# SunYangtian/UniGeo

Measured on AMD Instinct MI355X. Metric: frames/sec (384x512, 25-frame clip, 25 denoise steps), higher is better.
Workload: dtype fp16; 1 GPU; DepthCrafter SVD-UNet fp16, 25-step Euler, 25-frame 384x512 clips (BASELINE configs[1]); CLIP + VAE enc/dec + depth post-proc inside the timed region; one clip per ug_dc_run call, one call at a time (SURVEY 8d; reference eval.py:33-39); frames=25, height=384, width=512, denoise_steps=25, parallelism=clip-sharded x1, RCCL all_gather of depth, clips_in_flight_per_gpu=1, lanes=1

## Files before the change

### unigeo_amd/_lib.py

```python
import ctypes as C
import dataclasses
import json
import os

import numpy as np

_HERE = os.path.dirname(os.path.abspath(__file__))
LIB_PATH = os.environ.get("UG_LIB_PATH") or os.path.join(_HERE, "csrc", "libunigeo_hip.so")

EXPORTS = [
    "ug_unet_config_default", "ug_vae_config_default", "ug_clip_config_default",
    "ug_create", "ug_destroy", "ug_last_error", "ug_workspace_peak",
    "ug_load_tensor", "ug_bind_unet", "ug_bind_vae", "ug_bind_clip",
    "ug_dc_set_inputs", "ug_dc_run", "ug_dc_run_windows", "ug_dc_get_outputs", "ug_dc_device_ptrs", "ug_dc_set_trace", "ug_dc_set_guidance", "ug_unet_forward_pair", "ug_dc_set_inputs_ex", "ug_dc_get_noise", "ug_op_philox_u32", "ug_op_randn", "ug_op_u8_to_frames", "ug_set_vae_encode_fp32", "ug_set_concurrency", "ug_set_coscheduled", "ug_set_fp8_linears", "ug_op_linear_mx8", "ug_set_ff_fused", "ug_op_ff", "ug_op_ln_ff", "ug_bench_ff", "ug_bench_flash", "ug_tune_flash", "ug_tune_ff",
    "ug_eval_depth", "ug_eval_normal", "ug_depth_eval_opts_default", "ug_eval_depth_ex", "ug_eval_depth_global", "ug_op_masked_median", "ug_clip_embed", "ug_vae_encode", "ug_vae_decode", "ug_unet_forward", "ug_normals_from_depth",
    "ug_op_linear", "ug_op_conv", "ug_op_conv_gn", "ug_op_groupnorm", "ug_op_layernorm", "ug_op_flash_attn",
    "ug_op_temporal_attn", "ug_op_attention_generic", "ug_op_flash_attn_dh", "ug_op_euler_step", "ug_op_flash_cross_attn", "ug_op_temporal_attn_nv",
    "ug_op_split_pair", "ug_op_gn32_pair", "ug_op_conv_wide", "ug_op_attn_wide",
    "ug_bind_stablenormal", "ug_sn_run", "ug_sn_unet_forward", "ug_sn_dino", "ug_sn_vae_decode", "ug_sn_vae_encode", "ug_resize_bilinear",
    "ug_vis_depth_range", "ug_vis_panels", "ug_prep_resize_frames", "ug_prep_gt", "ug_prep_gt_ex",
    "ug_profile_begin", "ug_profile_begin_shapes", "ug_profile_end", "ug_bench_gemm", "ug_bench_groupnorm", "ug_bench_mfma_peak", "ug_tune_force",
]


class UNetConfigC(C.Structure):
    _fields_ = [("in_channels", C.c_int), ("out_channels", C.c_int), ("num_levels", C.c_int),
                ("block_out_channels", C.c_int * 8), ("num_attention_heads", C.c_int * 8),
                ("down_has_attn", C.c_int * 8),
                ("layers_per_block", C.c_int), ("cross_attention_dim", C.c_int),
                ("addition_time_embed_dim", C.c_int), ("projection_class_embeddings_input_dim", C.c_int),
                ("norm_groups", C.c_int),
# ... 89 lines not shown
    lib.ug_vae_decode.argtypes = [vp, vp, ip, ip, ip, vp]
    lib.ug_unet_forward.argtypes = [vp, vp, ip, ip, ip, C.c_float, vp, vp]
    lib.ug_normals_from_depth.argtypes = [vp, vp, vp, ip, ip, ip, vp]
    lib.ug_op_linear.argtypes = [vp, vp, ip, ip, vp, ip, vp, vp, C.c_float, C.c_float, ip, ip, vp]
    lib.ug_op_conv.argtypes = [vp, vp, ip, vp, ip, ip, ip, ip, vp, vp, ip, ip, ip, ip, ip, ip, ip, vp]
    lib.ug_op_groupnorm.argtypes = [vp, vp, ip, vp, ip, ip, ip, ip, C.c_float, ip, ip, vp, vp, vp]
    lib.ug_op_conv_gn.argtypes = [vp, vp, ip, ip, ip, ip, vp, vp, vp, ip, ip, ip, ip, C.c_float, ip, vp, vp, vp, vp, vp, vp]
    lib.ug_op_layernorm.argtypes = [vp, vp, ip, ip, C.c_float, vp, vp, vp, ip, vp, vp]
    lib.ug_op_flash_attn.argtypes = [vp, vp, ip, ip, ip, vp]
    lib.ug_op_temporal_attn.argtypes = [vp, vp, ip, ip, ip, vp]
    lib.ug_op_attention_generic.argtypes = [vp, vp, ip, ip, ip, ip, vp]
    lib.ug_op_flash_attn_dh.argtypes = [vp, vp, ip, ip, ip, ip, vp]
    lib.ug_op_euler_step.argtypes = [vp, vp, vp, C.c_long, C.c_float, C.c_float]
    _set_argtypes(lib, {"ug_op_flash_cross_attn": [vp, vp, vp, ip, ip, ip, ip, ip, C.c_long, C.c_long, C.c_long, C.c_long, vp],
                        "ug_op_temporal_attn_nv": [vp, vp, ip, ip, ip, ip, vp]})
    _set_argtypes(lib, {
        "ug_op_split_pair": [vp, vp, C.c_long, ip, vp, vp], "ug_op_gn32_pair": [vp, vp, ip, ip, ip, ip, C.c_float, ip, vp, vp, vp, vp],
        "ug_op_conv_wide": [vp, vp, ip, ip, ip, ip, vp, vp, ip, vp, ip, ip, ip, ip, ip, vp], "ug_op_attn_wide": [vp, vp, ip, ip, ip, vp]})
    lib.ug_bind_stablenormal.argtypes = [vp, C.POINTER(UNetConfigC), C.POINTER(VAEConfigC), C.POINTER(CLIPConfigC)]
    lib.ug_sn_run.argtypes = [vp, vp, ip, ip, ip, vp, C.c_float, ip, vp, vp, vp, vp]
    lib.ug_sn_unet_forward.argtypes = [vp, ip, vp, vp, ip, ip, ip, C.c_float, C.c_float, vp, vp, ip, vp]
    lib.ug_sn_dino.argtypes = [vp, vp, ip, ip, ip, vp]
    lib.ug_sn_vae_decode.argtypes = [vp, vp, ip, ip, ip, vp]
    lib.ug_sn_vae_encode.argtypes = [vp, vp, ip, ip, ip, vp]
    lib.ug_resize_bilinear.argtypes = [vp, vp, ip, ip, ip, ip, ip, ip, ip, vp]
    lib.ug_profile_begin.argtypes = [vp]
    lib.ug_bench_gemm.argtypes = [vp] + [ip] * 16 + [vp]
    lib.ug_bench_groupnorm.argtypes = [vp, ip, ip, ip, ip, ip, ip, ip, vp]
    lib.ug_bench_mfma_peak.argtypes = [vp, ip, vp]
    lib.ug_tune_force.argtypes = [vp, ip, ip]
# ... 496 lines not shown
        out = np.empty((M, N // 2 if geglu else N), np.float32)
        self._ck(self.lib.ug_op_linear(self.ctx, _ptr(A), M, K, _ptr(W), N, _ptr(b), _ptr(r), c0, c1, act, int(geglu), _ptr(out)))
        return out

    def op_conv(self, x0, weight, bias=None, x1=None, kt=1, k=3, stride=1, pad_t=1, pad_l=1, ups=1):
        x0 = _f32(x0); T, H, W, C0 = x0.shape
        x1a = None if x1 is None else _f32(x1); C1 = 0 if x1 is None else x1a.shape[-1]
        w = _f32(weight); O = w.shape[0]
        b = None if bias is None else _f32(bias)
        Ho, Wo = H * ups // stride, W * ups // stride
        out = np.empty((T, Ho, Wo, O), np.float32)
        self._ck(self.lib.ug_op_conv(self.ctx, _ptr(x0), C0, _ptr(x1a), C1, T, H, W, _ptr(w), _ptr(b), O, kt, k,
                                     stride, pad_t, pad_l, ups, _ptr(out)))
        return out

    def op_groupnorm(self, x0, G, eps, gamma, beta, x1=None, temporal=False, silu=False):
        x0 = _f32(x0); T, HW, C0 = x0.shape
        x1a = None if x1 is None else _f32(x1); C1 = 0 if x1 is None else x1a.shape[-1]
        out = np.empty((T, HW, C0 + C1), np.float32)
        self._ck(self.lib.ug_op_groupnorm(self.ctx, _ptr(x0), C0, _ptr(x1a), C1, T, HW, G, eps, int(temporal), int(silu),
                                          _ptr(_f32(gamma)), _ptr(_f32(beta)), _ptr(out)))
        return out

    def op_conv_gn(self, x, w, b, G, eps, gamma, beta, res=None, kt=1, k=3, temporal=False):
        x = _f32(x); T, H, W, C0 = x.shape; w = _f32(w); O = w.shape[0]
        r = None if res is None else _f32(res)
        co = np.empty((T, H, W, O), np.float32); y1 = np.empty_like(co); y2 = np.empty_like(co)
        rb = C.c_int(0)
        self._ck(self.lib.ug_op_conv_gn(self.ctx, _ptr(x), C0, T, H, W, _ptr(w), _ptr(None if b is None else _f32(b)), _ptr(r), O, kt, k, G, eps, int(temporal),
                                        _ptr(_f32(gamma)), _ptr(_f32(beta)), _ptr(co), _ptr(y1), _ptr(y2), C.byref(rb)))
# ... 109 lines not shown
```

### unigeo_amd/csrc/common.h

```cpp
#pragma once
#include <hip/hip_runtime.h>
#include <hip/hip_fp16.h>
#include <stdint.h>
#include <stdio.h>
#include <stdexcept>
#include <string>

typedef _Float16 f16;
typedef _Float16 f16x2 __attribute__((ext_vector_type(2)));
typedef _Float16 f16x4 __attribute__((ext_vector_type(4)));
typedef _Float16 f16x8 __attribute__((ext_vector_type(8)));
typedef float f32x4 __attribute__((ext_vector_type(4)));
typedef float f32x16 __attribute__((ext_vector_type(16)));

#define UG_CHECK(expr)                                                                        \
  do {                                                                                        \
    hipError_t _e = (expr);                                                                   \
    if (_e != hipSuccess)                                                                     \
      throw std::runtime_error(std::string(#expr) + " failed: " + hipGetErrorString(_e) +    \
                               " at " + __FILE__ + ":" + std::to_string(__LINE__));           \
  } while (0)

#define UG_REQUIRE(cond, msg)                                                                 \
  do {                                                                                        \
// ... 39 lines not shown
  int m_off;
  int group_m;
  int halo_tw, halo_lg;
  int tune_cfg_p1, tune_split_p1, tune_knobs;
  float2* stat_part; int stat_hw;
};
struct GemmTune { int cfg = -1, split = -1, knobs = 0; };
static inline void gemm_apply_tune(GemmP& p, const GemmTune& t) { p.tune_cfg_p1 = t.cfg + 1; p.tune_split_p1 = t.split + 1; p.tune_knobs = t.knobs; }
void launch_gemm_mx8(const GemmP& p, hipStream_t s);
void launch_quant_mx8(const f16* x, long ldx, long M, int K, unsigned char* q, unsigned* scales, long ld_s, hipStream_t s);
void launch_gemm(const GemmP& p, int batch, hipStream_t s, int* stat_rb = nullptr);
bool gemm_stream_supported(const GemmP& p, int batch);
void launch_gemm_stream(const GemmP& p, hipStream_t s);
bool conv_halo_supported(const GemmP& p, int batch, int bm, int bn);
void launch_conv_halo(const GemmP& p, int bm, int bn, hipStream_t s);
void gemm_plan(const GemmP& p, int batch, int* cfg_out, int* split_out);

struct FFusedP {
  const f16* X; const f16* W1; const f16* b1; const f16* W2; const f16* b2;
  const f16* R1; const f16* R2; float c0, c1, c2;
  f16* Out; int M, C; const f16* zero;
  const f16* ln_g; const f16* ln_b; float ln_eps; const f16* addvec; int rows_per_vec;
  int variant;
};
bool ff_fused_supported(int C);
void launch_ff_fused(const FFusedP& p, hipStream_t s);

struct GroupNormP {
  const f16* X0; const f16* X1; int C0, C1;
  int T, HW, G; float eps; int temporal; int silu;
// ... 131 lines not shown
```

### unigeo_amd/csrc/kernels/conv_halo.hip

```cpp
#include "gemm_common.h"
#include <algorithm>
#include <cstdlib>
#include <type_traits>

template <int BM, int BN, int LG, bool ST = false>
__global__ __launch_bounds__(12 * 64, 3) void conv_halo_kernel(const GemmP p) {
  constexpr int BK = 64, NCW = 8, WMW = 4, WNW = 2;
  constexpr unsigned SENT = 0x80000000u;
  constexpr int WTM = BM / WMW, WTN = BN / WNW;
  constexpr int MT = WTM / 16, NT = WTN / 16;
  constexpr int WID = 4 * NT;
  constexpr int LB = BN / 32;
  constexpr int WSLOT = BN * BK;
  constexpr int TW = 1 << LG, TH = BM >> LG;
  constexpr int PITCH = (TW + 2 + 7) & ~7;
  constexpr int GPR = PITCH / 8;
  constexpr int NG = (TH + 2) * GPR;
  constexpr int HALO = NG * 8 * BK;
  constexpr int HL = 2;
  constexpr int HSLOTS = 7 * HL;
  static_assert(TH * TW == BM && TW >= 16 && (NG + 3) / 4 <= HSLOTS, "tile geometry");
  static_assert((2 * HALO + 3 * WSLOT) * 2 <= 160 * 1024, "LDS");
  extern __shared__ __attribute__((aligned(16))) f16 smem[];
  f16* halo = smem;
  f16* ring = smem + 2 * HALO;

  const int tid = threadIdx.x, lane = tid & 63;
  const int wave = __builtin_amdgcn_readfirstlane(tid >> 6);
  const bool producer = wave >= NCW;
  const int ntn = (p.N + BN - 1) / BN, ntm = p.M / BM;
  const int ntiles = ntm * ntn;
  const int Cin = p.C0 + p.C1, nchunks = Cin / BK, nk = nchunks * 9;
  const int txn = p.Wo >> LG, tpf = (p.Ho / TH) * txn;

  const int nwg = gridDim.x, w = blockIdx.x;
  const TileWalk tw = tile_walk(p.flags, ntiles, nwg, w);
  const int my_tiles = tw.count;
  const int total_it = my_tiles * nk;

  auto tile_origin = [&](int tile, int& t, int& y0, int& x0, int& n0) {
    int tm, tn; tile_coord_p(p, tile, ntm, ntn, tm, tn);
    const int tmg = tm + p.m_off / BM;
    t = tmg / tpf;
    const int rem = tmg - t * tpf;
    const int tyi = rem / txn, txi = rem - tyi * txn;
    y0 = tyi * TH; x0 = txi * TW; n0 = tn * BN;
  };

  if (producer) {
    const int pw = wave - NCW;
    const int pc = lane & 7, lrow = lane >> 3;
    const int lc16_0 = (pc ^ ((0 + (lrow >> 1)) & 7)) * 16, lc16_1 = (pc ^ ((4 + (lrow >> 1)) & 7)) * 16;
    const int lc16_h = (pc ^ (((lrow >> 1) & 3) * 2)) * 16;
    const __amdgpu_buffer_rsrc_t rA0 = __builtin_amdgcn_make_buffer_rsrc((void*)p.A0, 0, (int)SENT, 0x00020000);
    const __amdgpu_buffer_rsrc_t rA1 = __builtin_amdgcn_make_buffer_rsrc((void*)(p.A1 ? p.A1 : p.A0), 0, (int)SENT, 0x00020000);
    const __amdgpu_buffer_rsrc_t rW = __builtin_amdgcn_make_buffer_rsrc((void*)p.W, 0, (int)SENT, 0x00020000);
    constexpr int ngw_max = (NG + 3) / 4;
    const int ngw = (NG - pw + 3) >> 2;
    int h_pix[HSLOTS];
    auto halo_setup = [&](int tile) {
      int t, y0, x0, n0; tile_origin(tile, t, y0, x0, n0);
#pragma unroll
      for (int k = 0; k < ngw_max; ++k) {
        const int grp = pw + 4 * k;
        const int hy = grp / GPR, hx = (grp - hy * GPR) * 8 + lrow;
        const int y = y0 - 1 + hy, x = x0 - 1 + hx;
        const bool ok = grp < NG && hx < TW + 2 && y >= 0 && y < p.Hi && x >= 0 && x < p.Wi;
        h_pix[k] = ok ? (t * p.Hi + y) * p.Wi + x : -1;
      }
    };
    auto halo_issue = [&](int k, int chunk, int hb) {
      const int cb = chunk * BK;
      const bool src0 = cb < p.C0;
      const int Cs2 = (src0 ? p.C0 : p.C1) * 2;
      const int soff = (src0 ? cb : cb - p.C0) * 2;
      const unsigned voff = h_pix[k] >= 0 ? (unsigned)h_pix[k] * (unsigned)Cs2 + (unsigned)lc16_h : SENT;
      __builtin_amdgcn_raw_ptr_buffer_load_lds(src0 ? rA0 : rA1, (lptr_t)(halo + hb * HALO + (pw + 4 * k) * 8 * BK), 16, (int)voff, soff, 0, 0);
    };
    unsigned b_off[LB];
    int ld_ti = 0, ld_ks = 0, ld_slot = 0;
// ... 6 lines not shown
        for (int l = 0; l < LB; ++l) {
          const int rg = pw * LB + l;
          const int lr = rg * 8 + lrow;
          const int part = lr / WTN, rem = lr % WTN;
          const int jj = rem >> 4, i = rem & 15;
          const int n = n0 + part * WTN + (i >> 2) * WID + jj * 4 + (i & 3);
          b_off[l] = n < p.N ? (unsigned)n * (unsigned)(p.ldw * 2) + ((rg & 1) ? lc16_1 : lc16_0) : SENT;
        }
      }
      f16* Bs = ring + ld_slot * WSLOT;
      const int kt2 = ld_ks * BK * 2;
#pragma unroll
      for (int l = 0; l < LB; ++l)
        __builtin_amdgcn_raw_ptr_buffer_load_lds(rW, (lptr_t)(Bs + (pw * LB + l) * 8 * BK), 16, (int)b_off[l], kt2, 0, 0);
      int nh = 0;
      const int chunk = ld_ks / 9, sp = ld_ks - chunk * 9;
      if (sp >= 2) {
        int tchunk = chunk + 1, ttile = ld_ti;
        if (tchunk == nchunks) { tchunk = 0; ++ttile; }
        if (ttile < my_tiles) {
          if (ttile != h_tile) { halo_setup(tw.first + ttile * tw.step); h_tile = ttile; }
#pragma unroll
          for (int u = 0; u < HL; ++u) {
            const int k = (sp - 2) * HL + u;
            if (k < ngw) {
#pragma unroll
              for (int kk = 0; kk < ngw_max; ++kk) if (kk == k) halo_issue(kk, tchunk, (ld_gc + 1) & 1);
              ++nh;
            }
          }
        }
      }
      if (++ld_ks == nk) { ld_ks = 0; ++ld_ti; }
      if (ld_ks % 9 == 0) ++ld_gc;
      if (++ld_slot == 3) ld_slot = 0;
      return nh;
    };
    if (total_it > 0) {
      halo_setup(tw.first); h_tile = 0;
#pragma unroll
      for (int k = 0; k < ngw_max; ++k) if (k < ngw) halo_issue(k, 0, 0);
      issue();
    }
    if (total_it > 1) issue();
    if (total_it > 1) asm volatile("s_waitcnt vmcnt(%0)" ::"n"(LB) : "memory");
    else asm volatile("s_waitcnt vmcnt(0)" ::: "memory");
    __builtin_amdgcn_s_barrier();
    for (int fi = 0; fi < total_it; ++fi) {
      if (fi + 2 < total_it) {
        const int nh = issue();
        if (nh == 2) asm volatile("s_waitcnt vmcnt(%0)" ::"n"(LB + 2) : "memory");
        else if (nh == 1) asm volatile("s_waitcnt vmcnt(%0)" ::"n"(LB + 1) : "memory");
        else asm volatile("s_waitcnt vmcnt(%0)" ::"n"(LB) : "memory");
      } else {
        asm volatile("s_waitcnt vmcnt(0)" ::: "memory");
      }
      __builtin_amdgcn_s_barrier();
    }
    return;
  }

  const int wm = wave / WNW, wn = wave % WNW;
  f32x4 acc[MT][NT];
#pragma unroll
  for (int i = 0; i < MT; ++i)
#pragma unroll
    for (int j = 0; j < NT; ++j) acc[i][j] = (f32x4){0.f, 0.f, 0.f, 0.f};
  const int l15 = lane & 15, g = lane >> 4;
  const int sw = swz<BK>(l15);
  const int r0 = wm * WTM;
  const int hpb = (r0 >> LG) * PITCH + (r0 & (TW - 1)) + l15;
  auto DI = [](int i) constexpr { return TW >= 64 ? i * 16 : TW == 32 ? (i >> 1) * PITCH + (i & 1) * 16 : i * PITCH; };
  static_assert(TW >= 64 || (TW == 32 && WTM % 32 == 0) || TW == 16, "row-block offsets");
  int a_pre[3][2], b_pre[2];
#pragma unroll
  for (int dx = 0; dx < 3; ++dx)
#pragma unroll
    for (int kk = 0; kk < 2; ++kk) {
      const int hp = hpb + dx;
      a_pre[dx][kk] = (hp * BK + (((kk * 4 + g) ^ (((hp >> 1) & 3) * 2)) * 8)) * 2;
    }
#pragma unroll
  for (int kk = 0; kk < 2; ++kk) b_pre[kk] = ((wn * WTN + l15) * BK + (((kk * 4 + g) ^ sw) * 8)) * 2;
  const char* ringb = (const char*)ring;
  int cp_ti = 0, cp_gc = 0;
  __builtin_amdgcn_s_barrier();
  asm volatile("" ::: "memory");
  const char* Hb = nullptr;
  int ti = 0;
  bool last_chunk = false;
  const bool lean = !ST && BN != 160 && tile_epilogue_lean_ok(p, WTN, true) && !(p.tune_knobs & 8388608);
  auto step = [&](auto TAP) {
    constexpr int tap = decltype(TAP)::value;
    constexpr int dy = tap / 3, dx = tap - dy * 3;
    constexpr int slot = tap % 3;
    {
      f16x8 af[2][MT], bf[2][NT];
#pragma unroll
      for (int kk = 0; kk < 2; ++kk) {
#pragma unroll
        for (int j = 0; j < NT; ++j) bf[kk][j] = *(const f16x8*)(ringb + b_pre[kk] + (slot * WSLOT + j * 16 * BK) * 2);
#pragma unroll
        for (int i = 0; i < MT; ++i) af[kk][i] = *(const f16x8*)(Hb + a_pre[dx][kk] + (dy * PITCH + DI(i)) * BK * 2);
      }
#pragma unroll
      for (int kk = 0; kk < 2; ++kk)
#pragma unroll
        for (int i = 0; i < MT; ++i)
#pragma unroll
          for (int j = 0; j < NT; ++j)
            acc[i][j] = __builtin_amdgcn_mfma_f32_16x16x32_f16(bf[kk][j], af[kk][i], acc[i][j], 0, 0, 0);
      constexpr int R = MT + NT, Q = MT * NT;
      __builtin_amdgcn_sched_group_barrier(0x100, R, 0);
#pragma unroll
      for (int r = 0; r < R; ++r) {
        __builtin_amdgcn_sched_group_barrier(0x008, Q / R, 0);
        __builtin_amdgcn_sched_group_barrier(0x100, 1, 0);
      }
      __builtin_amdgcn_sched_group_barrier(0x008, Q - R * (Q / R), 0);
      __builtin_amdgcn_sched_group_barrier(0x008, Q, 0);
    }
    asm volatile("s_waitcnt lgkmcnt(0)" ::: "memory");
    __builtin_amdgcn_s_barrier();
    asm volatile("" ::: "memory");
    if (tap == 8 && last_chunk) {
      int t, y0, x0, n0; tile_origin(tw.first + ti * tw.step, t, y0, x0, n0);
      const int m0 = (t * p.Ho + y0) * p.Wo + x0 - p.m_off;
      if constexpr (ST) tile_epilogue_stats<MT, NT, WTM, WTN>(p, acc, m0, n0, wm, wn, lane, (t * tpf + (y0 / TH) * txn + (x0 >> LG)) * (BM / WTM) + wm);
      else if constexpr (BN != 160) { if (lean) tile_epilogue_lean<MT, NT, WTM, WTN, false, true>(p, acc, m0, n0, wm, wn, lane, 0, nullptr); else tile_epilogue<MT, NT, WTM, WTN>(p, acc, m0, n0, wm, wn, lane, 0); }
      else tile_epilogue<MT, NT, WTM, WTN>(p, acc, m0, n0, wm, wn, lane, 0);
    }
  };
  for (ti = 0; ti < my_tiles; ++ti) {
    for (int c = 0; c < nchunks; ++c, ++cp_gc) {
      Hb = (const char*)(halo + (cp_gc & 1) * HALO);
      last_chunk = c == nchunks - 1;
      step(std::integral_constant<int, 0>{}); step(std::integral_constant<int, 1>{}); step(std::integral_constant<int, 2>{});
      step(std::integral_constant<int, 3>{}); step(std::integral_constant<int, 4>{}); step(std::integral_constant<int, 5>{});
      step(std::integral_constant<int, 6>{}); step(std::integral_constant<int, 7>{}); step(std::integral_constant<int, 8>{});
    }
  }
  (void)cp_ti;
}

static bool halo_geom_ok(const GemmP& p, int bm, int lg) {
  const int tw = 1 << lg, th = bm >> lg;
  if (th < 1 || th * tw != bm || p.Wo % tw || p.Ho % th) return false;
  const long band = (long)th * p.Wo;
  return p.m_off % band == 0 && p.M % band == 0;
}
static int halo_pick_lg(const GemmP& p, int bm, int bn) {
  if (bm == 256 && bn == 160) return halo_geom_ok(p, 256, 5) ? 5 : -1;
  if (bm == 256) { for (int lg : {4, 5, 6}) if (halo_geom_ok(p, 256, lg)) return lg; return -1; }
  return halo_geom_ok(p, 192, 4) ? 4 : -1;
// ... 30 lines not shown

void launch_conv_halo(const GemmP& p, int bm, int bn, hipStream_t s) {
  const int lg = halo_pick_lg(p, bm, bn);
  UG_REQUIRE(lg >= 0, "halo conv: no tile geometry");
  if (p.stat_part) {
    UG_REQUIRE(bn == 128, "halo conv: epilogue statistics on 128-column tiles only");
    if (bm == 192) launch_halo_t<192, 128, 4, true>(p, s);
    else if (lg == 4) launch_halo_t<256, 128, 4, true>(p, s); else if (lg == 5) launch_halo_t<256, 128, 5, true>(p, s); else launch_halo_t<256, 128, 6, true>(p, s);
    return;
  }
  if (bm == 256 && bn == 160) launch_halo_t<256, 160, 5>(p, s);
  else if (bm == 256) { if (lg == 4) launch_halo_t<256, 128, 4>(p, s); else if (lg == 5) launch_halo_t<256, 128, 5>(p, s); else launch_halo_t<256, 128, 6>(p, s); }
  else if (bn == 160) launch_halo_t<192, 160, 4>(p, s);
  else launch_halo_t<192, 128, 4>(p, s);
}
```

### unigeo_amd/csrc/kernels/gemm.hip

```cpp
#include "../common.h"
#include <algorithm>

#include "gemm_common.h"

template <int BM, int BN, int BK, int NST, int WMW, int WNW> struct GemmOcc {
  static constexpr int lds = NST * (BM + BN) * BK * 2;
  static constexpr int wg_lds = (160 * 1024) / lds;
  static constexpr int wg = wg_lds < 1 ? 1 : (wg_lds > 4 ? 4 : wg_lds);
  static constexpr int wps_raw = wg * WMW * WNW / 4;
  static constexpr int wps = wps_raw < 1 ? 1 : (wps_raw > 4 ? 4 : wps_raw);
};

#ifdef UG_GEMM_TRACE
#define UG_STAMP(slot)                                                                                   \
  do {                                                                                                   \
    if (traced && fi >= 8 && fi < 32) {                                                                  \
      unsigned long long c_;                                                                             \
      asm volatile("s_memtime %0\n\ts_waitcnt lgkmcnt(0)" : "=s"(c_)::"memory");                         \
      if (lane == 0) tr_lds[(fi - 8) * 5 + (slot)] = (unsigned)c_;                                       \
    }                                                                                                    \
  } while (0)
#else
#define UG_STAMP(slot) do {} while (0)
#endif
// ... 1025 lines not shown
    case 19: launch_mode<256, 128, 64, 3, 2, 4>(p, batch, s); break;
    case 35: if (gemm_can_bufa(p, 64, true)) launch_ldr<256, 256, 2, 2, 4>(p, batch, s); else launch_mode<256, 256, 64, 2, 2, 4>(p, batch, s); break;
    case 39: if (gemm_can_bufa(p, 64, true)) launch_ldr<256, 128, 3, 2, 4>(p, batch, s); else launch_mode<256, 128, 64, 3, 2, 4>(p, batch, s); break;
    case 59: if (gemm_can_bufa(p, 64, true)) launch_ws<128, 2, 4>(p, batch, s); else launch_mode<256, 128, 64, 3, 2, 4>(p, batch, s); break;
    case 54: if (gemm_can_bufa(p, 64, true)) launch_ws<128, 4, 2>(p, batch, s); else launch_mode<256, 128, 64, 3, 4, 2>(p, batch, s); break;
    case 60: if (gemm_can_bufa(p, 64, true)) launch_ws<160, 4, 2>(p, batch, s); else launch_mode<256, 64, 64, 2, 4, 2>(p, batch, s); break;
    case 34: if (gemm_can_bufa(p, 64, true)) launch_ldr<256, 64, 2, 4, 2>(p, batch, s); else launch_mode<256, 64, 64, 2, 4, 2>(p, batch, s); break;
    case 61: launch_mode<192, 128, 64, 3, 2, 4>(p, batch, s); break;
    case 62: launch_mode<192, 128, 64, 3, 4, 2>(p, batch, s); break;
    case 63: if (gemm_can_bufa(p, 64, true)) launch_ws<128, 2, 4, 192>(p, batch, s); else launch_mode<192, 128, 64, 3, 2, 4>(p, batch, s); break;
    case 64: if (gemm_can_bufa(p, 64, true)) launch_ws<128, 4, 2, 192>(p, batch, s); else launch_mode<192, 128, 64, 3, 4, 2>(p, batch, s); break;
    case 70: UG_REQUIRE(conv_halo_supported(p, batch, 256, 160), "config 70: not a halo-stageable convolution"); launch_conv_halo(p, 256, 160, s); break;
    case 71: UG_REQUIRE(conv_halo_supported(p, batch, 256, 128), "config 71: not a halo-stageable convolution"); launch_conv_halo(p, 256, 128, s); break;
    case 72: UG_REQUIRE(conv_halo_supported(p, batch, 192, 128), "config 72: not a halo-stageable convolution"); launch_conv_halo(p, 192, 128, s); break;
    case 73: UG_REQUIRE(conv_halo_supported(p, batch, 192, 160), "config 73: not a halo-stageable convolution"); launch_conv_halo(p, 192, 160, s); break;
    case 80: launch_gemm_stream(p, s); break;
    default: UG_REQUIRE(false, "unknown / pruned GEMM tile config");
  }
}

template <int BM, int BN, int NST, int WMW, int WNW, bool BUFA>
static void launch_mx_t(const GemmP& p, hipStream_t s) {
  const int ntiles = cdiv(p.M, BM) * cdiv(p.N, BN);
  const size_t lds = (size_t)NST * (BM + BN) * 64 * sizeof(f16) + (size_t)NST * (BM + BN) * 4;
  auto kern = gemm_kernel<BM, BN, 64, NST, WMW, WNW, false, false, BUFA, true>;
  static bool attr[32] = {};
  bool& at = attr[ug_dev_slot()];
  if (!at) { UG_CHECK(hipFuncSetAttribute((const void*)kern, hipFuncAttributeMaxDynamicSharedMemorySize, (int)lds)); at = true; }
  const int per_cu = std::max(1, std::min(2, (int)((160 * 1024) / lds)));
  int gx = (per_cu * 256 / 8) * 8;
// ... 170 lines not shown
}

static bool cfg_geom(int cfg, int& bm, int& bn, int& wmw, int& wnw) {
  switch (cfg) {
    case 0: bm = 128; bn = 128; wmw = 2; wnw = 2; return true;
    case 1: case 3: bm = 128; bn = 64; wmw = 2; wnw = 2; return true;
    case 4: case 8: case 54: bm = 256; bn = 128; wmw = 4; wnw = 2; return true;
    case 12: bm = 64; bn = 64; wmw = 2; wnw = 2; return true;
    case 14: case 34: bm = 256; bn = 64; wmw = 4; wnw = 2; return true;
    case 15: case 35: bm = 256; bn = 256; wmw = 2; wnw = 4; return true;
    case 19: case 39: case 59: bm = 256; bn = 128; wmw = 2; wnw = 4; return true;
    case 61: case 63: bm = 192; bn = 128; wmw = 2; wnw = 4; return true;
    case 62: case 64: bm = 192; bn = 128; wmw = 4; wnw = 2; return true;
    default: return false;
  }
}

void launch_gemm(const GemmP& p0, int batch, hipStream_t s, int* stat_rb) {
  GemmP p = p0;
  if (stat_rb) *stat_rb = 0;
  if (!stat_rb) p.stat_part = nullptr;
  if (p.tune_knobs & 2) p.flags |= UG_F_NOXCD;
  if (p.tune_knobs & 128) p.flags |= UG_F_XCDROUND;
  if (p.tune_knobs & 16) p.flags |= UG_F_PRIO;
  UG_REQUIRE(p.K % 8 == 0, "GEMM K must be a multiple of 8");
  UG_REQUIRE(p.ldw % 8 == 0, "GEMM ldw must be a multiple of 8");
  UG_REQUIRE(p.M > 0 && p.N > 0 && p.K > 0, "empty GEMM");
  UG_REQUIRE(p.zero != nullptr, "zero page missing");
  UG_REQUIRE(p.nb_inner >= 1, "nb_inner");
  if (p.flags & UG_F_GEGLU) UG_REQUIRE(p.N % 128 == 0, "GEGLU GEMM needs N % 128 == 0");
// ... 40 lines not shown
  }
  if (halo_on) {
    int best = -1; double bfill = 0.0;
    for (int c = 70; c <= 73; ++c) {
      const int bm = c <= 71 ? 256 : 192, bn = (c == 70 || c == 73) ? 160 : 128;
      if (!conv_halo_supported(p, batch, bm, bn)) continue;
      const long tiles = (long)(p.M / bm) * cdiv(p.N, bn);
      const double useful = (double)p.N / (cdiv(p.N, bn) * bn);
      const double fill = (double)tiles / (cdiv(tiles, 256) * 256.0) * useful * (bm == 256 ? 1.0 : 0.97);
      if (fill > bfill) { bfill = fill; best = c; }
    }
    if (halo_l0) best = 71;
    else if (p.N % 160 == 0 && p.N <= 320) best = -1;
    if (best >= 0) cfg = best;
  }
  if (planned && !(p.tune_knobs & 65536) && (p.tune_cfg_p1 - 1) < 0 && split == 1 && gemm_stream_supported(p, batch)) {
    cfg = 80;
  }
  if (split > 1) UG_REQUIRE(p.partial != nullptr, "split-K needs a partial buffer");
  p.group_m = pick_group_m(p, cfg, batch, split);
  p.tm_T = p.tm_nb = 0;
  if (p.conv && p.kt > 1 && p.T > 1 && batch == 1 && !(p.tune_knobs & 256)) {
    int bm = 256;
    switch (cfg) { case 0: case 1: case 3: bm = 128; break; case 12: bm = 64; break; case 61: case 62: case 63: case 64: bm = 192; break; default: break; }
    const long hw = (long)p.Ho * p.Wo;
    if (hw % bm == 0 && hw / bm >= 1) { p.tm_T = p.T; p.tm_nb = (int)(hw / bm); }
  }
  if (p.stat_part) {
    int bm = 0, wmw = 0;
    {
      int gbm, gbn, gwm, gwn;
      const bool sym = (cfg == 14 || cfg == 19) && p.conv && gemm_can_bufa(p, 64, false) && !(p.tune_knobs & 4);
      const bool pk = (cfg == 35 || cfg == 54 || cfg == 59 || cfg == 63 || cfg == 64) && p.conv && gemm_can_bufa(p, 64, true);
      if (cfg == 71) { bm = 256; wmw = 4; }
      else if (cfg == 72) { bm = 192; wmw = 4; }
      else if ((sym || pk) && cfg_geom(cfg, gbm, gbn, gwm, gwn)) { bm = gbm; wmw = gwm; }
    }
    const int wtm = bm ? bm / wmw : 0;
    const bool ok = bm && split == 1 && batch == 1 && !(p.flags & (UG_F_GEGLU | UG_F_OUT_F32 | UG_F_R1_F32)) && !p.up_phase && !(p.tune_knobs & 131072) &&
                    p.M % bm == 0 && p.m_off == 0 && p.stat_hw > 0 && p.stat_hw % wtm == 0 && p.N % 16 == 0 && p.ldo % 8 == 0 &&
                    (!p.R1 || p.ldr1 % 8 == 0) && (!p.R2 || p.ldr2 % 8 == 0);
    static const bool sdbg = getenv("UG_STAT_DEBUG") != nullptr;
    if (sdbg) fprintf(stderr, "[stat] M %d N %d K %d conv %d kt %d hw %d cfg %d split %d -> rb %d\n", p.M, p.N, p.K, p.conv, p.kt, p.stat_hw, cfg, split, ok ? wtm : 0);
    if (ok) *stat_rb = wtm; else p.stat_part = nullptr;
  }
  launch_cfg(cfg, p, batch, s);
  if (split > 1) {
    const long nvec = (long)p.M * (p.N / 8);
    int grid = (int)std::min<long>((nvec + 255) / 256, 256 * 8);
    hipLaunchKernelGGL(splitk_epilogue, dim3(grid), dim3(256), 0, s, p);
  }
  UG_CHECK(hipGetLastError());
}
```

### unigeo_amd/csrc/kernels/gemm_common.h

```cpp
#pragma once
#include "../common.h"
#include <type_traits>

typedef const __attribute__((address_space(1))) void* gptr_t;
typedef __attribute__((address_space(3))) void* lptr_t;

__device__ __forceinline__ float erf_as(float x) {
  const float ax = fabsf(x);
  const float t = __frcp_rn(1.0f + 0.3275911f * ax);
  const float y = ((((1.061405429f * t - 1.453152027f) * t + 1.421413741f) * t - 0.284496736f) * t + 0.254829592f) * t;
  const float r = 1.0f - y * __expf(-ax * ax);
  return copysignf(r, x);
}
__device__ __forceinline__ float gelu_f(float x) { return 0.5f * x * (1.0f + erf_as(x * 0.70710678118654752f)); }
__device__ __forceinline__ float silu_f(float x) { return x * __builtin_amdgcn_rcpf(1.0f + __expf(-x)); }

typedef float f32x2 __attribute__((ext_vector_type(2)));
__device__ __forceinline__ f32x2 geglu2(f32x2 h, f32x2 g) {
  const f32x2 ag = {__builtin_fabsf(g.x), __builtin_fabsf(g.y)};
  const f32x2 u = ag * 0.23164189f + 1.0f;
  const f32x2 t = {__builtin_amdgcn_rcpf(u.x), __builtin_amdgcn_rcpf(u.y)};
  f32x2 y = t * 0.5307027145f - 0.7265760135f;
  y = y * t + 0.7107068705f;
  y = y * t - 0.142248368f;
// ... 358 lines not shown
      asm("" : "+v"(r));
      h[e] = (f16)r.x; h[e + 1] = (f16)r.y;
    }
    if (in && m < p.M) *(f16x8*)(Ob + (long)m * p.ldo) = h;
  }
}

__device__ __forceinline__ float row16_sum(float x) {
  x += __builtin_bit_cast(float, __builtin_amdgcn_update_dpp(0, __builtin_bit_cast(int, x), 0xB1, 0xf, 0xf, true));
  x += __builtin_bit_cast(float, __builtin_amdgcn_update_dpp(0, __builtin_bit_cast(int, x), 0x4E, 0xf, 0xf, true));
  x += __builtin_bit_cast(float, __builtin_amdgcn_update_dpp(0, __builtin_bit_cast(int, x), 0x141, 0xf, 0xf, true));
  x += __builtin_bit_cast(float, __builtin_amdgcn_update_dpp(0, __builtin_bit_cast(int, x), 0x140, 0xf, 0xf, true));
  return x;
}

template <int MT, int NT, int WTM, int WTN>
__device__ __forceinline__ void tile_epilogue_stats(const GemmP& p, f32x4 (&acc)[MT][NT], int m0, int n0, int wm, int wn, int lane, int stat_blk) {
  constexpr int WID = 4 * NT;
  static_assert(WID % 8 == 0, "statistics epilogue: 8-column chunks");
  static_assert(WID <= 16, "statistics epilogue: a lane's WID-column run is stored whole or not at all - launch_gemm only guarantees N % 16 == 0");
  const int l15 = lane & 15, g = lane >> 4;
  const int nb = n0 + wn * WTN + g * WID;
  const bool full = (nb + WID <= p.N);
  auto body = [&](auto MODE_) {
  constexpr int MODE = decltype(MODE_)::value;
#pragma unroll
  for (int e = 0; e < WID; e += 8) {
    float bv[8];
#pragma unroll
    for (int q = 0; q < 8; ++q) bv[q] = 0.f;
    if (full) {
      if (p.bias) { const f16x8 b = *(const f16x8*)(p.bias + nb + e);
#pragma unroll
        for (int q = 0; q < 8; ++q) bv[q] += (float)b[q]; }
      if (p.bias2) { const f16x8 b = *(const f16x8*)(p.bias2 + nb + e);
#pragma unroll
        for (int q = 0; q < 8; ++q) bv[q] += (float)b[q]; }
    }
    float ssum[8], ssq[8];
#pragma unroll
    for (int q = 0; q < 8; ++q) { ssum[q] = 0.f; ssq[q] = 0.f; }
#pragma unroll
    for (int i = 0; i < MT; ++i) {
      int m = m0 + wm * WTM + i * 16 + l15;
      if (p.halo_tw) { const int r = wm * WTM + i * 16 + l15; m = m0 + (r >> p.halo_lg) * p.Wo + (r & (p.halo_tw - 1)); }
      float o[8];
#pragma unroll
      for (int q = 0; q < 8; ++q) {
        if constexpr (MODE == 0) o[q] = p.c0 * (acc[i][(e + q) >> 2][(e + q) & 3] + bv[q]);
        else o[q] = acc[i][(e + q) >> 2][(e + q) & 3] + bv[q];
        acc[i][(e + q) >> 2][(e + q) & 3] = 0.f;
      }
      if (!full) continue;
      if (MODE == 1 || (MODE == 0 && p.R1)) {
        const f16x8 r = *(const f16x8*)(p.R1 + (long)m * p.ldr1 + nb + e);
#pragma unroll
        for (int q = 0; q < 8; ++q) o[q] += p.c1 * (float)r[q];
      }
      if constexpr (MODE == 0) {
        if (p.R2) {
          const f16x8 r = *(const f16x8*)(p.R2 + (long)m * p.ldr2 + nb + e);
#pragma unroll
          for (int q = 0; q < 8; ++q) o[q] += p.c2 * (float)r[q];
        }
        if (p.act == UG_ACT_SILU) {
#pragma unroll
          for (int q = 0; q < 8; ++q) o[q] = silu_f(o[q]);
        } else if (p.act == UG_ACT_GELU) {
#pragma unroll
          for (int q = 0; q < 8; ++q) o[q] = gelu_f(o[q]);
// ... 27 lines not shown
```

Baseline: 27.81 frames/s.

## Add halo-staged temporal (kt=3) convolution kernel with statistics epilogue

```diff
diff --git a/unigeo_amd/_lib.py b/unigeo_amd/_lib.py
--- a/unigeo_amd/_lib.py
+++ b/unigeo_amd/_lib.py
@@ -14,7 +14,7 @@
     "ug_load_tensor", "ug_bind_unet", "ug_bind_vae", "ug_bind_clip",
     "ug_dc_set_inputs", "ug_dc_run", "ug_dc_run_windows", "ug_dc_get_outputs", "ug_dc_device_ptrs", "ug_dc_set_trace", "ug_dc_set_guidance", "ug_unet_forward_pair", "ug_dc_set_inputs_ex", "ug_dc_get_noise", "ug_op_philox_u32", "ug_op_randn", "ug_op_u8_to_frames", "ug_set_vae_encode_fp32", "ug_set_concurrency", "ug_set_coscheduled", "ug_set_fp8_linears", "ug_op_linear_mx8", "ug_set_ff_fused", "ug_op_ff", "ug_op_ln_ff", "ug_bench_ff", "ug_bench_flash", "ug_tune_flash", "ug_tune_ff",
     "ug_eval_depth", "ug_eval_normal", "ug_depth_eval_opts_default", "ug_eval_depth_ex", "ug_eval_depth_global", "ug_op_masked_median", "ug_clip_embed", "ug_vae_encode", "ug_vae_decode", "ug_unet_forward", "ug_normals_from_depth",
-    "ug_op_linear", "ug_op_conv", "ug_op_conv_gn", "ug_op_groupnorm", "ug_op_layernorm", "ug_op_flash_attn",
+    "ug_op_linear", "ug_op_conv", "ug_op_conv_epi", "ug_op_conv_gn", "ug_op_groupnorm", "ug_op_layernorm", "ug_op_flash_attn",
     "ug_op_temporal_attn", "ug_op_attention_generic", "ug_op_flash_attn_dh", "ug_op_euler_step", "ug_op_flash_cross_attn", "ug_op_temporal_attn_nv",
     "ug_op_split_pair", "ug_op_gn32_pair", "ug_op_conv_wide", "ug_op_attn_wide",
     "ug_bind_stablenormal", "ug_sn_run", "ug_sn_unet_forward", "ug_sn_dino", "ug_sn_vae_decode", "ug_sn_vae_encode", "ug_resize_bilinear",
@@ -134,6 +134,7 @@
     lib.ug_op_euler_step.argtypes = [vp, vp, vp, C.c_long, C.c_float, C.c_float]
     _set_argtypes(lib, {"ug_op_flash_cross_attn": [vp, vp, vp, ip, ip, ip, ip, ip, C.c_long, C.c_long, C.c_long, C.c_long, vp],
                         "ug_op_temporal_attn_nv": [vp, vp, ip, ip, ip, ip, vp]})
+    _set_argtypes(lib, {"ug_op_conv_epi": [vp, vp, ip, ip, ip, ip, vp, vp, vp, vp, C.c_float, C.c_float, ip, ip, ip, vp]})
     _set_argtypes(lib, {
         "ug_op_split_pair": [vp, vp, C.c_long, ip, vp, vp], "ug_op_gn32_pair": [vp, vp, ip, ip, ip, ip, C.c_float, ip, vp, vp, vp, vp],
         "ug_op_conv_wide": [vp, vp, ip, ip, ip, ip, vp, vp, ip, vp, ip, ip, ip, ip, ip, vp], "ug_op_attn_wide": [vp, vp, ip, ip, ip, vp]})
@@ -660,6 +661,13 @@
                                      stride, pad_t, pad_l, ups, _ptr(out)))
         return out
 
+    def op_conv_epi(self, x, weight, bias=None, bias2=None, res=None, c0=1.0, c1=1.0, kt=1, k=3):
+        x = _f32(x); T, H, W, C0 = x.shape; w = _f32(weight); O = w.shape[0]
+        opt = lambda a: None if a is None else _f32(a)
+        out = np.empty((T, H, W, O), np.float32)
+        self._ck(self.lib.ug_op_conv_epi(self.ctx, _ptr(x), C0, T, H, W, _ptr(w), _ptr(opt(bias)), _ptr(opt(bias2)), _ptr(opt(res)), c0, c1, O, kt, k, _ptr(out)))
+        return out
+
     def op_groupnorm(self, x0, G, eps, gamma, beta, x1=None, temporal=False, silu=False):
         x0 = _f32(x0); T, HW, C0 = x0.shape
         x1a = None if x1 is None else _f32(x1); C1 = 0 if x1 is None else x1a.shape[-1]
diff --git a/unigeo_amd/csrc/common.h b/unigeo_amd/csrc/common.h
--- a/unigeo_amd/csrc/common.h
+++ b/unigeo_amd/csrc/common.h
@@ -77,6 +77,8 @@
 void launch_gemm_stream(const GemmP& p, hipStream_t s);
 bool conv_halo_supported(const GemmP& p, int batch, int bm, int bn);
 void launch_conv_halo(const GemmP& p, int bm, int bn, hipStream_t s);
+bool tconv_halo_supported(const GemmP& p, int batch, int bn, int lg);
+void launch_tconv_halo(const GemmP& p, int bn, int lg, hipStream_t s);
 void gemm_plan(const GemmP& p, int batch, int* cfg_out, int* split_out);
 
 struct FFusedP {
diff --git a/unigeo_amd/csrc/kernels/conv_halo.hip b/unigeo_amd/csrc/kernels/conv_halo.hip
--- a/unigeo_amd/csrc/kernels/conv_halo.hip
+++ b/unigeo_amd/csrc/kernels/conv_halo.hip
@@ -3,7 +3,7 @@
 #include <cstdlib>
 #include <type_traits>
 
-template <int BM, int BN, int LG, bool ST = false>
+template <int BM, int BN, int LG, bool ST = false, bool TC = false>
 __global__ __launch_bounds__(12 * 64, 3) void conv_halo_kernel(const GemmP p) {
   constexpr int BK = 64, NCW = 8, WMW = 4, WNW = 2;
   constexpr unsigned SENT = 0x80000000u;
@@ -13,13 +13,15 @@
   constexpr int LB = BN / 32;
   constexpr int WSLOT = BN * BK;
   constexpr int TW = 1 << LG, TH = BM >> LG;
-  constexpr int PITCH = (TW + 2 + 7) & ~7;
+  constexpr int NTAP = TC ? 3 : 9;
+  constexpr int PITCH = TC ? TW : (TW + 2 + 7) & ~7;
   constexpr int GPR = PITCH / 8;
   constexpr int NG = (TH + 2) * GPR;
   constexpr int HALO = NG * 8 * BK;
-  constexpr int HL = 2;
-  constexpr int HSLOTS = 7 * HL;
+  constexpr int HL = TC ? ((NG + 3) / 4 + 1) / 2 : 2;
+  constexpr int HSLOTS = (TC ? 2 : 7) * HL;
   static_assert(TH * TW == BM && TW >= 16 && (NG + 3) / 4 <= HSLOTS, "tile geometry");
+  static_assert(!TC || !ST || TW == BM / WMW, "temporal statistics blocks: a wave's rows are one run of one frame");
   static_assert((2 * HALO + 3 * WSLOT) * 2 <= 160 * 1024, "LDS");
   extern __shared__ __attribute__((aligned(16))) f16 smem[];
   f16* halo = smem;
@@ -28,10 +30,10 @@
   const int tid = threadIdx.x, lane = tid & 63;
   const int wave = __builtin_amdgcn_readfirstlane(tid >> 6);
   const bool producer = wave >= NCW;
-  const int ntn = (p.N + BN - 1) / BN, ntm = p.M / BM;
+  const int txn = p.Wo >> LG, tpf = (p.Ho / TH) * txn;
+  const int ntn = (p.N + BN - 1) / BN, ntm = TC ? ((p.T + TH - 1) / TH) * txn : p.M / BM;
   const int ntiles = ntm * ntn;
-  const int Cin = p.C0 + p.C1, nchunks = Cin / BK, nk = nchunks * 9;
-  const int txn = p.Wo >> LG, tpf = (p.Ho / TH) * txn;
+  const int Cin = p.C0 + p.C1, nchunks = Cin / BK, nk = nchunks * NTAP;
 
   const int nwg = gridDim.x, w = blockIdx.x;
   const TileWalk tw = tile_walk(p.flags, ntiles, nwg, w);
@@ -40,6 +42,7 @@
 
   auto tile_origin = [&](int tile, int& t, int& y0, int& x0, int& n0) {
     int tm, tn; tile_coord_p(p, tile, ntm, ntn, tm, tn);
+    if constexpr (TC) { const int tf = tm / txn; t = tf * TH; y0 = 0; x0 = (tm - tf * txn) * TW; n0 = tn * BN; return; }
     const int tmg = tm + p.m_off / BM;
     t = tmg / tpf;
     const int rem = tmg - t * tpf;
@@ -64,6 +67,11 @@
       for (int k = 0; k < ngw_max; ++k) {
         const int grp = pw + 4 * k;
         const int hy = grp / GPR, hx = (grp - hy * GPR) * 8 + lrow;
+        if constexpr (TC) {
+          const int f = t - 1 + hy;
+          h_pix[k] = (grp < NG && f >= 0 && f < p.T) ? f * p.Wi + x0 + hx : -1;
+          continue;
+        }
         const int y = y0 - 1 + hy, x = x0 - 1 + hx;
         const bool ok = grp < NG && hx < TW + 2 && y >= 0 && y < p.Hi && x >= 0 && x < p.Wi;
         h_pix[k] = ok ? (t * p.Hi + y) * p.Wi + x : -1;
@@ -100,8 +108,21 @@
       for (int l = 0; l < LB; ++l)
         __builtin_amdgcn_raw_ptr_buffer_load_lds(rW, (lptr_t)(Bs + (pw * LB + l) * 8 * BK), 16, (int)b_off[l], kt2, 0, 0);
       int nh = 0;
-      const int chunk = ld_ks / 9, sp = ld_ks - chunk * 9;
-      if (sp >= 2) {
+      const int chunk = ld_ks / NTAP, sp = ld_ks - chunk * NTAP;
+      if constexpr (TC) {
+        if (sp == 0 && ld_gc > 0) {
+#pragma unroll
+          for (int u = 0; u < HL; ++u) {
+            const int k = HL + u;
+            if (k < ngw) {
+#pragma unroll
+              for (int kk = 0; kk < ngw_max; ++kk) if (kk == k) halo_issue(kk, chunk, ld_gc & 1);
+              ++nh;
+            }
+          }
+        }
+      }
+      if (TC ? sp == 2 : sp >= 2) {
         int tchunk = chunk + 1, ttile = ld_ti;
         if (tchunk == nchunks) { tchunk = 0; ++ttile; }
         if (ttile < my_tiles) {
@@ -118,7 +139,7 @@
         }
       }
       if (++ld_ks == nk) { ld_ks = 0; ++ld_ti; }
-      if (ld_ks % 9 == 0) ++ld_gc;
+      if (ld_ks % NTAP == 0) ++ld_gc;
       if (++ld_slot == 3) ld_slot = 0;
       return nh;
     };
@@ -135,7 +156,12 @@
     for (int fi = 0; fi < total_it; ++fi) {
       if (fi + 2 < total_it) {
         const int nh = issue();
-        if (nh == 2) asm volatile("s_waitcnt vmcnt(%0)" ::"n"(LB + 2) : "memory");
+        static_assert(HL <= 6, "halo slices per step");
+        if (TC && nh == 6) asm volatile("s_waitcnt vmcnt(%0)" ::"n"(LB + 6) : "memory");
+        else if (TC && nh == 5) asm volatile("s_waitcnt vmcnt(%0)" ::"n"(LB + 5) : "memory");
+        else if (TC && nh == 4) asm volatile("s_waitcnt vmcnt(%0)" ::"n"(LB + 4) : "memory");
+        else if (TC && nh == 3) asm volatile("s_waitcnt vmcnt(%0)" ::"n"(LB + 3) : "memory");
+        else if (nh == 2) asm volatile("s_waitcnt vmcnt(%0)" ::"n"(LB + 2) : "memory");
         else if (nh == 1) asm volatile("s_waitcnt vmcnt(%0)" ::"n"(LB + 1) : "memory");
         else asm volatile("s_waitcnt vmcnt(%0)" ::"n"(LB) : "memory");
       } else {
@@ -156,8 +182,8 @@
   const int sw = swz<BK>(l15);
   const int r0 = wm * WTM;
   const int hpb = (r0 >> LG) * PITCH + (r0 & (TW - 1)) + l15;
-  auto DI = [](int i) constexpr { return TW >= 64 ? i * 16 : TW == 32 ? (i >> 1) * PITCH + (i & 1) * 16 : i * PITCH; };
-  static_assert(TW >= 64 || (TW == 32 && WTM % 32 == 0) || TW == 16, "row-block offsets");
+  auto DI = [](int i) constexpr { return TC ? i * 16 : TW >= 64 ? i * 16 : TW == 32 ? (i >> 1) * PITCH + (i & 1) * 16 : i * PITCH; };
+  static_assert(TC || TW >= 64 || (TW == 32 && WTM % 32 == 0) || TW == 16, "row-block offsets");
   int a_pre[3][2], b_pre[2];
 #pragma unroll
   for (int dx = 0; dx < 3; ++dx)
@@ -178,7 +204,7 @@
   const bool lean = !ST && BN != 160 && tile_epilogue_lean_ok(p, WTN, true) && !(p.tune_knobs & 8388608);
   auto step = [&](auto TAP) {
     constexpr int tap = decltype(TAP)::value;
-    constexpr int dy = tap / 3, dx = tap - dy * 3;
+    constexpr int dy = TC ? tap : tap / 3, dx = TC ? 0 : tap - dy * 3;
     constexpr int slot = tap % 3;
     {
       f16x8 af[2][MT], bf[2][NT];
@@ -209,10 +235,19 @@
     asm volatile("s_waitcnt lgkmcnt(0)" ::: "memory");
     __builtin_amdgcn_s_barrier();
     asm volatile("" ::: "memory");
-    if (tap == 8 && last_chunk) {
+    if (tap == NTAP - 1 && last_chunk) {
       int t, y0, x0, n0; tile_origin(tw.first + ti * tw.step, t, y0, x0, n0);
       const int m0 = (t * p.Ho + y0) * p.Wo + x0 - p.m_off;
-      if constexpr (ST) tile_epilogue_stats<MT, NT, WTM, WTN>(p, acc, m0, n0, wm, wn, lane, (t * tpf + (y0 / TH) * txn + (x0 >> LG)) * (BM / WTM) + wm);
+      if constexpr (TC && ST) {
+        if (t + wm < p.T) tile_epilogue_stats<MT, NT, WTM, WTN, true>(p, acc, m0, n0, wm, wn, lane, ((t + wm) * p.Wo + x0) / WTM);
+        else {
+#pragma unroll
+          for (int i = 0; i < MT; ++i)
+#pragma unroll
+            for (int j = 0; j < NT; ++j) acc[i][j] = (f32x4){0.f, 0.f, 0.f, 0.f};
+        }
+      }
+      else if constexpr (ST) tile_epilogue_stats<MT, NT, WTM, WTN>(p, acc, m0, n0, wm, wn, lane, (t * tpf + (y0 / TH) * txn + (x0 >> LG)) * (BM / WTM) + wm);
       else if constexpr (BN != 160) { if (lean) tile_epilogue_lean<MT, NT, WTM, WTN, false, true>(p, acc, m0, n0, wm, wn, lane, 0, nullptr); else tile_epilogue<MT, NT, WTM, WTN>(p, acc, m0, n0, wm, wn, lane, 0); }
       else tile_epilogue<MT, NT, WTM, WTN>(p, acc, m0, n0, wm, wn, lane, 0);
     }
@@ -222,8 +257,10 @@
       Hb = (const char*)(halo + (cp_gc & 1) * HALO);
       last_chunk = c == nchunks - 1;
       step(std::integral_constant<int, 0>{}); step(std::integral_constant<int, 1>{}); step(std::integral_constant<int, 2>{});
-      step(std::integral_constant<int, 3>{}); step(std::integral_constant<int, 4>{}); step(std::integral_constant<int, 5>{});
-      step(std::integral_constant<int, 6>{}); step(std::integral_constant<int, 7>{}); step(std::integral_constant<int, 8>{});
+      if constexpr (!TC) {
+        step(std::integral_constant<int, 3>{}); step(std::integral_constant<int, 4>{}); step(std::integral_constant<int, 5>{});
+        step(std::integral_constant<int, 6>{}); step(std::integral_constant<int, 7>{}); step(std::integral_constant<int, 8>{});
+      }
     }
   }
   (void)cp_ti;
@@ -284,3 +321,45 @@
   else if (bn == 160) launch_halo_t<192, 160, 4>(p, s);
   else launch_halo_t<192, 128, 4>(p, s);
 }
+
+bool tconv_halo_supported(const GemmP& p, int batch, int bn, int lg) {
+  if (!p.conv || batch != 1 || p.kt != 3 || p.ky != 1 || p.kx != 1 || p.stride != 1 || p.ups != 1 || p.pad_t != 0 || p.pad_l != 0) return false;
+  if (!p.kchunk || p.up_phase || p.splitk > 1 || p.Hi != p.Ho || p.Wi != p.Wo || p.m_off != 0) return false;
+  if (p.flags & (UG_F_GEGLU | UG_F_OUT_F32)) return false;
+  if (p.C1 != 0 || p.C0 % 64 || p.N % 16 || p.T < 4 || lg < 4 || lg > 6 || bn != 128) return false;
+  const long hw = (long)p.Ho * p.Wo;
+  if (hw % (1 << lg) || p.M != p.T * hw) return false;
+  const long lim = (1L << 31) - 64;
+  const long rows = (long)(p.T + (256 >> lg)) * hw;
+  return rows * std::max(p.C0, p.N) * 2 < lim && (long)p.N * p.ldw * 2 < lim;
+}
+
+template <int BN, int LG, bool ST = false>
+static void launch_thalo_t(const GemmP& p, hipStream_t s) {
+  constexpr int BM = 256, TW = 1 << LG, TH = BM >> LG, NG = (TH + 2) * (TW / 8);
+  const size_t lds = 2 * (size_t)NG * 1024 + 3 * (size_t)BN * 128;
+  static bool attr[32] = {};
+  bool& at = attr[ug_dev_slot()];
+  if (!at) {
+    UG_CHECK(hipFuncSetAttribute((const void*)conv_halo_kernel<BM, BN, LG, ST, true>, hipFuncAttributeMaxDynamicSharedMemorySize, 160 * 1024));
+    at = true;
+  }
+  const int hw = p.Ho * p.Wo;
+  const int ntiles = cdiv(p.T, TH) * (hw / TW) * cdiv(p.N, BN);
+  const int gx = std::min(256, ntiles);
+  static const bool dbg = getenv("UG_HALO_DEBUG") != nullptr;
+  if (dbg) fprintf(stderr, "[halo-t] 256x%d T %d HW %d N %d C %d  tile %d frames x %d px  lds %zu  grid %d  stats %d\n", BN, p.T, hw, p.N, p.C0, TH, TW, lds, gx, (int)ST);
+  GemmP q = p; q.halo_lg = LG; q.halo_tw = TW; q.splitk = 1; q.Hi = q.Ho = 1; q.Wi = q.Wo = hw; q.tm_T = q.tm_nb = 0;
+  hipLaunchKernelGGL((conv_halo_kernel<BM, BN, LG, ST, true>), dim3(gx), dim3(12 * 64), lds, s, q);
+}
+
+void launch_tconv_halo(const GemmP& p, int bn, int lg, hipStream_t s) {
+  if (p.stat_part) {
+    UG_REQUIRE(bn == 128 && lg == 6, "temporal halo conv: epilogue statistics on 4 x 64 tiles of 128 columns only");
+    launch_thalo_t<128, 6, true>(p, s);
+    return;
+  }
+  if (lg == 6) launch_thalo_t<128, 6>(p, s);
+  else if (lg == 5) launch_thalo_t<128, 5>(p, s);
+  else launch_thalo_t<128, 4>(p, s);
+}
diff --git a/unigeo_amd/csrc/kernels/gemm.hip b/unigeo_amd/csrc/kernels/gemm.hip
--- a/unigeo_amd/csrc/kernels/gemm.hip
+++ b/unigeo_amd/csrc/kernels/gemm.hip
@@ -1063,6 +1063,7 @@
     case 71: UG_REQUIRE(conv_halo_supported(p, batch, 256, 128), "config 71: not a halo-stageable convolution"); launch_conv_halo(p, 256, 128, s); break;
     case 72: UG_REQUIRE(conv_halo_supported(p, batch, 192, 128), "config 72: not a halo-stageable convolution"); launch_conv_halo(p, 192, 128, s); break;
     case 73: UG_REQUIRE(conv_halo_supported(p, batch, 192, 160), "config 73: not a halo-stageable convolution"); launch_conv_halo(p, 192, 160, s); break;
+    case 75: case 76: case 77: UG_REQUIRE(tconv_halo_supported(p, batch, 128, 81 - cfg), "config 75 - 77: not a halo-stageable temporal convolution"); launch_tconv_halo(p, 128, 81 - cfg, s); break;
     case 80: launch_gemm_stream(p, s); break;
     default: UG_REQUIRE(false, "unknown / pruned GEMM tile config");
   }
@@ -1263,6 +1264,23 @@
     case 62: case 64: bm = 192; bn = 128; wmw = 4; wnw = 2; return true;
     default: return false;
   }
+}
+
+static int tconv_halo_pick(const GemmP& p, int batch, bool stats) {
+  int best = -1; long bcost = 0;
+  for (int c = 75; c <= 77; ++c) {
+    const int bn = 128, lg = 81 - c;
+    if (stats && c != 75) continue;
+    if (!tconv_halo_supported(p, batch, bn, lg)) continue;
+    const long tw = 1 << lg, th = 256 >> lg, hw = (long)p.Ho * p.Wo;
+    const long tiles = (long)cdiv(p.T, th) * (hw / tw) * cdiv(p.N, bn);
+    const long cost = (long)cdiv(tiles, 256) * ((th + 2) * tw + 3 * bn);
+    if (best < 0 || cost < bcost) { best = c; bcost = cost; }
+  }
+  return best;
+}
+static bool tconv_halo_adopt(const GemmP& p) {
+  return p.M >= 50000 && p.N <= 320;
 }
 
 void launch_gemm(const GemmP& p0, int batch, hipStream_t s, int* stat_rb) {
@@ -1333,6 +1351,10 @@
     else if (p.N % 160 == 0 && p.N <= 320) best = -1;
     if (best >= 0) cfg = best;
   }
+  if (planned && !(p.tune_knobs & 33554432) && (p.tune_cfg_p1 - 1) < 0 && split == 1) {
+    const int tc = tconv_halo_pick(p, batch, p.stat_part != nullptr);
+    if (tc >= 0 && (tconv_halo_adopt(p) || (p.tune_knobs & 67108864))) cfg = tc;
+  }
   if (planned && !(p.tune_knobs & 65536) && (p.tune_cfg_p1 - 1) < 0 && split == 1 && gemm_stream_supported(p, batch)) {
     cfg = 80;
   }
@@ -1351,13 +1373,13 @@
       int gbm, gbn, gwm, gwn;
       const bool sym = (cfg == 14 || cfg == 19) && p.conv && gemm_can_bufa(p, 64, false) && !(p.tune_knobs & 4);
       const bool pk = (cfg == 35 || cfg == 54 || cfg == 59 || cfg == 63 || cfg == 64) && p.conv && gemm_can_bufa(p, 64, true);
-      if (cfg == 71) { bm = 256; wmw = 4; }
+      if (cfg == 71 || cfg == 75) { bm = 256; wmw = 4; }
       else if (cfg == 72) { bm = 192; wmw = 4; }
       else if ((sym || pk) && cfg_geom(cfg, gbm, gbn, gwm, gwn)) { bm = gbm; wmw = gwm; }
     }
     const int wtm = bm ? bm / wmw : 0;
     const bool ok = bm && split == 1 && batch == 1 && !(p.flags & (UG_F_GEGLU | UG_F_OUT_F32 | UG_F_R1_F32)) && !p.up_phase && !(p.tune_knobs & 131072) &&
-                    p.M % bm == 0 && p.m_off == 0 && p.stat_hw > 0 && p.stat_hw % wtm == 0 && p.N % 16 == 0 && p.ldo % 8 == 0 &&
+                    (p.M % bm == 0 || cfg == 75) && p.m_off == 0 && p.stat_hw > 0 && p.stat_hw % wtm == 0 && p.N % 16 == 0 && p.ldo % 8 == 0 &&
                     (!p.R1 || p.ldr1 % 8 == 0) && (!p.R2 || p.ldr2 % 8 == 0);
     static const bool sdbg = getenv("UG_STAT_DEBUG") != nullptr;
     if (sdbg) fprintf(stderr, "[stat] M %d N %d K %d conv %d kt %d hw %d cfg %d split %d -> rb %d\n", p.M, p.N, p.K, p.conv, p.kt, p.stat_hw, cfg, split, ok ? wtm : 0);
diff --git a/unigeo_amd/csrc/kernels/gemm_common.h b/unigeo_amd/csrc/kernels/gemm_common.h
--- a/unigeo_amd/csrc/kernels/gemm_common.h
+++ b/unigeo_amd/csrc/kernels/gemm_common.h
@@ -396,7 +396,7 @@
   return x;
 }
 
-template <int MT, int NT, int WTM, int WTN>
+template <int MT, int NT, int WTM, int WTN, bool RB = false>
 __device__ __forceinline__ void tile_epilogue_stats(const GemmP& p, f32x4 (&acc)[MT][NT], int m0, int n0, int wm, int wn, int lane, int stat_blk) {
   constexpr int WID = 4 * NT;
   static_assert(WID % 8 == 0, "statistics epilogue: 8-column chunks");
@@ -419,6 +419,17 @@
 #pragma unroll
         for (int q = 0; q < 8; ++q) bv[q] += (float)b[q]; }
     }
+    f16x8 rr[MT];
+    if constexpr (RB) {
+      if (full && (MODE == 1 || (MODE == 0 && p.R1))) {
+#pragma unroll
+        for (int i = 0; i < MT; ++i) {
+          int m = m0 + wm * WTM + i * 16 + l15;
+          if (p.halo_tw) { const int r = wm * WTM + i * 16 + l15; m = m0 + (r >> p.halo_lg) * p.Wo + (r & (p.halo_tw - 1)); }
+          rr[i] = *(const f16x8*)(p.R1 + (long)m * p.ldr1 + nb + e);
+        }
+      }
+    }
     float ssum[8], ssq[8];
 #pragma unroll
     for (int q = 0; q < 8; ++q) { ssum[q] = 0.f; ssq[q] = 0.f; }
@@ -435,7 +446,8 @@
       }
       if (!full) continue;
       if (MODE == 1 || (MODE == 0 && p.R1)) {
-        const f16x8 r = *(const f16x8*)(p.R1 + (long)m * p.ldr1 + nb + e);
+        f16x8 r;
+        if constexpr (RB) r = rr[i]; else r = *(const f16x8*)(p.R1 + (long)m * p.ldr1 + nb + e);
 #pragma unroll
         for (int q = 0; q < 8; ++q) o[q] += p.c1 * (float)r[q];
       }
```

Result: no change. 27.88 frames/s (median of 6 runs) (+0.3%).
